# fims9000/SYNT_ISIC

Hardware: AMD Instinct MI355X
Metric: images/sec at 3x64x64 T=1000 (DDPM reverse-diffusion sampling) (higher is better)
Workload: dtype f32

## Files before the change

### synt_isic_amd/csrc/common.h

```cpp
#pragma once

#include <hip/hip_runtime.h>

#include <atomic>
#include <cstdarg>
#include <cstdint>
#include <cstdio>
#include <string>
#include <map>
#include <mutex>
#include <vector>

#include "../../include/sisic.h"

namespace sisic {

void set_error(const char* fmt, ...);

#define SISIC_HIP(call)                                                                   \
    do {                                                                                  \
        hipError_t _e = (call);                                                           \
        if (_e != hipSuccess) {                                                           \
            ::sisic::set_error("%s failed: %s (%s:%d)", #call, hipGetErrorString(_e),     \
                               __FILE__, __LINE__);                                       \
// ... 41 lines not shown
    std::map<hipStream_t, SplitK> splitk;
    std::mutex splitk_mutex;
    struct Bf3Items { int key[9]; unsigned* tab = nullptr; hipStream_t fill_stream = nullptr; hipEvent_t fill_done = nullptr; };
    std::vector<Bf3Items> bf3_items;
    std::mutex bf3_items_mutex;
    std::atomic<uint64_t> scratch_generation{0};
};

namespace sisic {

struct ProfileScope {
    sisic_ctx* ctx;
    hipStream_t stream;
    PendingEvent ev{};
    bool active = false;
    ProfileScope(sisic_ctx* c, hipStream_t s, int kind, double bytes, double flops, double flops_exec = -1.0, int kind2 = -1);
    ~ProfileScope();
};

int profile_collect(sisic_ctx* ctx);

inline int ensure_dynamic_lds(sisic_ctx* ctx, const void* kern, int bytes, std::atomic<uint64_t>& done) {
    const uint64_t bit = uint64_t(1) << (ctx->device & 63);
    if (done.load(std::memory_order_acquire) & bit) return SISIC_OK;
    SISIC_HIP(hipFuncSetAttribute(kern, hipFuncAttributeMaxDynamicSharedMemorySize, bytes));
    done.fetch_or(bit, std::memory_order_release);
    return SISIC_OK;
}

inline int cdiv(int a, int b) { return (a + b - 1) / b; }
inline int wino_latency_ksplit(int Cout, int Cin, int Hout, int Wout) {
    const int co_t = Cout > 64 ? 128 : 64;
    const int per_image = cdiv(Hout, 8) * cdiv(Wout, 16) * cdiv(Cout, co_t);
    const int nchunks = cdiv(Cin, 8);
    int k = 1;
    while (per_image * k < 256 && k < 8 && nchunks % (2 * k) == 0) k *= 2;
    return k;
}
inline int wino_latency_segments(int Hout, int Wout) { return cdiv(Hout * Wout, 1024); }
inline int64_t cdiv64(int64_t a, int64_t b) { return (a + b - 1) / b; }
inline int round_up(int a, int b) { return cdiv(a, b) * b; }

constexpr int CONV_CO_TILE = 64;
inline int conv_ci_chunk(int ksize) { return ksize == 1 ? 32 : (ksize == 3 ? 16 : 4); }
inline int conv_cin_pad(int cin, int ksize) { return round_up(cin, conv_ci_chunk(ksize)); }
inline int conv_cout_pad(int cout) { return round_up(cout, CONV_CO_TILE); }
inline int64_t conv_packed_floats(int cout, int cin, int ksize) {
    const int64_t first = (int64_t)conv_cin_pad(cin, ksize) * ksize * ksize * conv_cout_pad(cout);
    return ksize == 1 ? 3 * first + first / 2 : first;
}

int launch_conv2d(sisic_ctx*, const sisic_conv_args& a, hipStream_t s);
int launch_conv_smallcout(sisic_ctx*, const sisic_conv_args& a, hipStream_t s);
int launch_score_head_bwd(sisic_ctx*, const float* logits, const float* fc_w, const float* act, float* g, int B, int C,
                          int HW, int n_classes, int target, hipStream_t s);
int launch_relu_bwd(sisic_ctx*, const float* dy, const float* y, float* out, int64_t n, hipStream_t s);
int launch_scatter_add_even(sisic_ctx*, float* dst, const float* src, int planes, int H, int W, hipStream_t s);
int launch_maxpool_bwd(sisic_ctx*, const float* dm, const float* xin, float* dx, int planes, int H, int W, hipStream_t s);
int launch_stem_bwd(sisic_ctx*, const float* g, const float* w_oihw, float* dp, int B, int CO, int OH, int OW, int H, int W,
                    hipStream_t s);
int launch_preprocess_bwd(sisic_ctx*, const float* dp, const float* x, float* dx, int B, int H, int W, int OH, int OW,
                          hipStream_t s);
int launch_add_relu(sisic_ctx*, const float* y, const float* identity, float* out, int64_t n, hipStream_t s);
int launch_gradcam(sisic_ctx*, const float* y, const float* outp, const float* fc_w, const float* bias, float* cam, int B, int C,
                   int h, int w, int S, int target, hipStream_t s);
int conv_stats_slots(const sisic_conv_args& a);
bool conv_finalizes(const sisic_conv_args& a);
bool conv_pointwise_applicable(const sisic_conv_args& a);
int conv_pointwise_stats_slots(const sisic_conv_args& a);
int launch_conv_pointwise(sisic_ctx*, const sisic_conv_args& a, hipStream_t s);
bool conv_pointwise_bf3_applicable(const sisic_conv_args& a);
int launch_conv_pointwise_bf3(sisic_ctx*, const sisic_conv_args& a, hipStream_t s);
bool conv_s2_bf3_applicable(const sisic_conv_args& a);
int conv_s2_bf3_stats_slots(const sisic_conv_args& a);
int launch_conv_s2_bf3(sisic_ctx*, const sisic_conv_args& a, hipStream_t s);
int64_t conv_s2_packed_floats(int Cout, int Cin);
int launch_conv_s2_pack(sisic_ctx*, const float* w, int Cout, int Cin, float* out, hipStream_t s);
int launch_gn_finalize(sisic_ctx*, const float* st0, int c0, int slots0, const float* st1, int c1, int slots1, int B,
                       int HW, int groups, float eps, const float* gamma, const float* beta, float* scale, float* shift,
                       hipStream_t s, float* mean_rstd = nullptr);
int launch_conv_winograd(sisic_ctx*, const sisic_conv_args& a, const float* u_packed, int cfg, hipStream_t s);
int launch_winograd_pack(sisic_ctx*, const float* w, int Cout, int Cin, float* packed, hipStream_t s);
int64_t winograd_packed_numel(int Cout, int Cin);
inline int64_t winograd_first_floats(int Cout, int Cin) { return (int64_t)round_up(Cin, 16) * 16 * conv_cout_pad(Cout); }
int launch_conv_pack(sisic_ctx*, const float* w, int Cout, int Cin, int k, float* packed, hipStream_t s);
int launch_gn_stats(sisic_ctx*, const float* in0, int c0, const float* in1, int c1, int B, int HW, int groups,
                    float eps, const float* gamma, const float* beta, float* scale, float* shift, hipStream_t s,
                    float* mean_rstd = nullptr);
int launch_attention(sisic_ctx*, const float* qkv, float* out, int B, int C, int N, int head_dim, hipStream_t s);
int launch_ddpm_step(sisic_ctx*, const float* eps, const float* x, const float* z, float* out, int64_t n,
                     float sb, float sa, float c0, float c1, float sigma, float clip, hipStream_t s);
size_t loop_state_bytes();
int launch_loop_select_row(sisic_ctx*, const float* table, int R, const void* state, float* out, hipStream_t s);
int launch_loop_advance(sisic_ctx*, void* state, hipStream_t s);
int launch_ddpm_step_indexed(sisic_ctx*, const float* eps, float* x, int64_t n, const void* state, const float* coef,
                             const int* zrow, float clip, hipStream_t s);
int launch_ddpm_step_rng(sisic_ctx*, const float* eps, const float* x, float* out, int64_t n, int64_t n_per_image,
                         const uint64_t* seeds_dev, uint32_t step, float sb, float sa, float c0, float c1, float sigma,
                         float clip, hipStream_t s);
int launch_ddpm_step_indexed_rng(sisic_ctx*, const float* eps, float* x, int64_t n, int64_t n_per_image, const void* state,
                                 const float* coef, const uint64_t* seeds_dev, float clip, hipStream_t s);
int launch_noise_fill(sisic_ctx*, void* out, int B, int64_t n_per_image, const uint64_t* seeds_host, uint32_t step,
                      uint32_t tag, bool bits, hipStream_t s);
int launch_denorm_u8(sisic_ctx*, const float* x, uint8_t* out, int B, int C, int H, int W, hipStream_t s, int form = 0);
int launch_temb_mlp(sisic_ctx*, const float* t_vals, int B, const float* freqs, int n_freqs, const float* w1t,
                    const float* b1, const float* w2t, const float* b2, int hidden, float* temb_act, hipStream_t s,
// ... 29 lines not shown
```

### synt_isic_amd/csrc/conv_mfma.hip

```cpp
#include <cstdlib>
#include <type_traits>

#include "common.h"
#include "pack_device.h"

namespace sisic {

typedef float f32x16 __attribute__((ext_vector_type(16)));

struct ConvParams {
    const float* in0;
    const float* in1;
    int c0, c1;
    int B, Hin, Win;
    int Hc, Wc;
    int Hout, Wout;
    int ups;
    int zero_insert;
    const float* w;
    int cout_pad;
    const float* bias;
    int Cout;
    const float* gn_scale;
    const float* gn_shift;
// ... 354 lines not shown
                                 float* __restrict__ out) {
    const size_t first = (size_t)cin_pad * KK * cout_pad;
    const size_t total = KK == 1 ? 3 * first + first / 2 : first;
    for (size_t i = (size_t)blockIdx.x * blockDim.x + threadIdx.x; i < total; i += (size_t)gridDim.x * blockDim.x) {
        conv_pack_elem(i, w, Cout, Cin, KK, cin_pad, cout_pad, out);
    }
}

template <int KS, int STRIDE, int MT, int NT, int WM, int WN, int TW, int CIC, int OCC = 2, int KSP = 1>
static int launch_cfg(sisic_ctx* ctx, ConvParams& p, hipStream_t s) {
    using G = ConvGeom<KS, STRIDE, MT, NT, WM, WN, TW, CIC, KSP>;
    p.tiles_x = cdiv(p.Wout, TW);
    p.tiles_y = cdiv(p.Hout, G::TH);
    p.n_co_tiles = p.cout_pad / G::CO_TILE;
    p.nchunks = cdiv(p.c0 + p.c1, CIC);
    const int64_t nwg = (int64_t)p.B * p.tiles_x * p.tiles_y * p.n_co_tiles;
    SISIC_REQUIRE(nwg > 0 && nwg < (int64_t(1) << 31), "conv2d: grid of %lld workgroups unsupported", (long long)nwg);
    p.nwg = (int)nwg;
    if (p.slots_query) {
        *p.slots_query = p.tiles_x * p.tiles_y * WN;
        return SISIC_OK;
    }
    if constexpr (KS == 1 && STRIDE == 1 && TW == G::PIX && G::EPT % 4 == 0) {
        const bool aligned = ((reinterpret_cast<uintptr_t>(p.in0) | reinterpret_cast<uintptr_t>(p.in1)) & 15) == 0;
        if (p.Wc % 4 == 0 && aligned) {
            auto kern4 = conv_mfma_kernel<KS, STRIDE, MT, NT, WM, WN, TW, CIC, OCC, KSP, true>;
            static std::atomic<uint64_t> lds_opt_in4{0};
            SISIC_TRY(ensure_dynamic_lds(ctx, reinterpret_cast<const void*>(kern4), (int)G::LDS_BYTES, lds_opt_in4));
            hipLaunchKernelGGL(kern4, dim3(p.nwg), dim3(G::NTHR), G::LDS_BYTES, s, p);
            SISIC_HIP(hipGetLastError());
            return SISIC_OK;
        }
    }
    auto kern = conv_mfma_kernel<KS, STRIDE, MT, NT, WM, WN, TW, CIC, OCC, KSP>;
    static std::atomic<uint64_t> lds_opt_in{0};
    SISIC_TRY(ensure_dynamic_lds(ctx, reinterpret_cast<const void*>(kern), (int)G::LDS_BYTES, lds_opt_in));
    hipLaunchKernelGGL(kern, dim3(p.nwg), dim3(G::NTHR), G::LDS_BYTES, s, p);
    SISIC_HIP(hipGetLastError());
    return SISIC_OK;
}

int launch_conv_pack(sisic_ctx*, const float* w, int Cout, int Cin, int k, float* packed, hipStream_t s) {
    SISIC_REQUIRE(k == 1 || k == 3 || k == 7, "conv_pack: ksize %d unsupported", k);
    const int cin_pad = conv_cin_pad(Cin, k), cout_pad = conv_cout_pad(Cout);
    const size_t total = (size_t)cin_pad * k * k * cout_pad;
    const int blocks = (int)std::min<size_t>((total * (k == 1 ? 4 : 1) + 255) / 256, 4096);
    hipLaunchKernelGGL(conv_pack_kernel, dim3(blocks), dim3(256), 0, s, w, Cout, Cin, k * k, cin_pad, cout_pad, packed);
    SISIC_HIP(hipGetLastError());
    return SISIC_OK;
}

static int dispatch_conv2d(sisic_ctx* ctx, const sisic_conv_args& a, hipStream_t s, int* slots_query);

static int winograd_cfg(const sisic_conv_args& a) {
    if (!(a.ksize == 3 && a.stride == 1 && a.w_winograd != nullptr && a.Cout > 4) || a.upsample == 2) return 0;
    if ((a.tile_cfg >= 60 && a.tile_cfg <= 74) || a.tile_cfg == 78 || a.tile_cfg == 79 || (a.tile_cfg >= 90 && a.tile_cfg <= 92)) return a.tile_cfg;
    if (a.tile_cfg != 0) return 0;
    const int Hout = a.Hin << (a.upsample ? 1 : 0), Wout = a.Win << (a.upsample ? 1 : 0);
    const bool fits32 = 16.0 * std::max(a.c0, a.c1) * a.Hin * a.Win < 4294967296.0;
    if (!fits32) return 0;
    if (Hout >= 12 && Wout >= 12) {
        static const bool wide_on = [] { const char* e = std::getenv("SISIC_WINO_WIDE"); return !e || std::atoi(e) != 0; }();
        static const bool bf3_on = [] { const char* e = std::getenv("SISIC_WINO_BF16X3"); return !e || std::atoi(e) != 0; }();
        const int th = (Hout + 15) / 16 * 16, tw = (Wout + 15) / 16 * 16;
        if (bf3_on && a.Cout % 64 == 0 && 4 * Hout * Wout >= 3 * th * tw && a.c0 + a.c1 >= 16 &&
            a.c0 + a.c1 <= 2048 &&
            4.0 * a.Cout * Hout * Wout < 2147483648.0)
            return 74;
        if (wide_on && !a.upsample) return a.Cout > 64 ? 68 : 69;
        return 66;
    }
    const int Cin = a.c0 + a.c1;
    static const bool ksplit_on = [] { const char* e = std::getenv("SISIC_KSPLIT"); return !e || std::atoi(e) != 0; }();
    if (ksplit_on && Hout <= 8 && Wout <= 8 && Hout >= 5 && Wout >= 5 && Cin >= 128 && Cin % 32 == 0 && a.Cout >= 128) {
        static const bool wide_on = [] { const char* e = std::getenv("SISIC_WINO_WIDE"); return !e || std::atoi(e) != 0; }();
        static const bool bf3_on = [] { const char* e = std::getenv("SISIC_WINO_BF16X3"); return !e || std::atoi(e) != 0; }();
        if (bf3_on && !a.upsample && a.Cout % 64 == 0 && Cin <= 512) return 92;
        return (wide_on && !a.upsample) ? 91 : 90;
    }
    return 0;
}
static bool winograd_selected(const sisic_conv_args& a) { return winograd_cfg(a) != 0; }

int conv_stats_slots(const sisic_conv_args& a) {
    if (const int cfg = winograd_cfg(a)) {
        if (cfg >= 90 && cfg <= 92) return 1;
        const int Hout = a.Hin << (a.upsample ? 1 : 0), Wout = a.Win << (a.upsample ? 1 : 0);
        if ((cfg == 78 || cfg == 79) && wino_latency_ksplit(a.Cout, a.c0 + a.c1, Hout, Wout) > 1) return wino_latency_segments(Hout, Wout);
        if ((cfg >= 68 && cfg <= 73) || cfg == 78 || cfg == 79) return ((Hout + 7) / 8) * ((Wout + 15) / 16);
        const int edge = (cfg == 61 || cfg == 63 || cfg == 65 || cfg == 67) ? 8 : 16;
        return ((Hout + edge - 1) / edge) * ((Wout + edge - 1) / edge);
    }
    int slots = 0;
    sisic_conv_args q = a;
    q.stats_out = nullptr;
    if (dispatch_conv2d(nullptr, q, nullptr, &slots) != SISIC_OK) return 0;
    return slots;
}

bool conv_finalizes(const sisic_conv_args& a) {
    if (!a.fin_gamma || a.fin_groups <= 0) return false;
    const int cfg = winograd_cfg(a);
    const int Hout = a.Hin << (a.upsample ? 1 : 0), Wout = a.Win << (a.upsample ? 1 : 0);
    if (a.Cout % a.fin_groups != 0 || a.Cout / a.fin_groups != 8) return false;
    if (cfg == 74) return !a.upsample && Hout <= 16 && Wout <= 16 && a.Cout % 64 == 0;
    if (cfg < 90 || cfg > 92) return false;
    if (Hout * Wout != 64 || a.Cout % 16 != 0) return false;
    return ((reinterpret_cast<uintptr_t>(a.residual) | reinterpret_cast<uintptr_t>(a.out) | reinterpret_cast<uintptr_t>(a.stats_out)) & 15) == 0;
}

int launch_conv2d(sisic_ctx* ctx, const sisic_conv_args& a, hipStream_t s) { return dispatch_conv2d(ctx, a, s, nullptr); }

static int dispatch_conv2d(sisic_ctx* ctx, const sisic_conv_args& a, hipStream_t s, int* slots_query) {
    SISIC_REQUIRE(a.in0 && a.w_packed && a.out, "conv2d: null tensor");
    SISIC_REQUIRE(a.B > 0 && a.Hin > 0 && a.Win > 0 && a.c0 > 0 && a.c1 >= 0 && a.Cout > 0, "conv2d: bad shape");
    SISIC_REQUIRE((a.c1 == 0) == (a.in1 == nullptr), "conv2d: in1/c1 mismatch");
    SISIC_REQUIRE(a.ksize == 1 || a.ksize == 3 || a.ksize == 7, "conv2d: ksize %d unsupported", a.ksize);
    SISIC_REQUIRE(a.stride == 1 || a.stride == 2, "conv2d: stride %d unsupported", a.stride);
    SISIC_REQUIRE(a.ksize != 7 || a.stride == 2, "conv2d: 7x7 is built for stride 2 only (the ResNet stem)");
    SISIC_REQUIRE(!(a.upsample && a.stride != 1), "conv2d: upsample with stride");
    SISIC_REQUIRE((a.gn_scale == nullptr) == (a.gn_shift == nullptr), "conv2d: gn_scale/gn_shift mismatch");

    ConvParams p{};
    p.in0 = a.in0; p.in1 = a.in1; p.c0 = a.c0; p.c1 = a.c1;
    p.B = a.B; p.Hin = a.Hin; p.Win = a.Win;
    p.ups = a.upsample ? 1 : 0;
    p.zero_insert = a.upsample == 2 ? 1 : 0;
    p.Hc = a.Hin << p.ups; p.Wc = a.Win << p.ups;
    const int pad = a.ksize / 2;
    p.Hout = (p.Hc + 2 * pad - a.ksize) / a.stride + 1;
    p.Wout = (p.Wc + 2 * pad - a.ksize) / a.stride + 1;
    p.w = a.w_packed; p.cout_pad = conv_cout_pad(a.Cout);
    p.bias = a.bias; p.Cout = a.Cout;
    p.gn_scale = a.gn_scale; p.gn_shift = a.gn_shift; p.gn_silu = a.gn_silu;
    p.chan_bias = a.chan_bias; p.chan_bias_stride = a.chan_bias_stride; p.residual = a.residual; p.relu = a.relu; p.out = a.out;
    p.stats = a.stats_out; p.slots_query = slots_query;

    const int Cin = a.c0 + a.c1;
    const double kk = double(a.ksize) * a.ksize;
    const double out_elems = double(a.B) * a.Cout * p.Hout * p.Wout;
    const double bytes = 4.0 * (double(a.B) * Cin * a.Hin * a.Win + out_elems) + 4.0 * (Cin * a.Cout * kk + a.Cout) +
                         (a.residual ? 4.0 * out_elems : 0.0);
    const double flops = 2.0 * out_elems * Cin * kk;
    int cfg = a.tile_cfg;
    const bool use_wino = winograd_selected(a);
    SISIC_REQUIRE(a.stats_out == nullptr || conv_stats_slots(a) > 0,
                  "conv2d: stats_out given but sisic_conv_stats_slots() is 0 for these arguments");
    const bool wino_ups9 = use_wino && a.upsample && !a.gn_scale && winograd_cfg(a) == 66;
    ProfileScope prof(slots_query ? nullptr : ctx, s, a.ksize == 1 ? PK_CONV1 : PK_CONV3, bytes, flops,
                      use_wino ? flops * (wino_ups9 ? 9.0 : 16.0) / 36.0 : flops,
                      (use_wino && winograd_cfg(a) == 74) ? PK_WINO_BF3 :
                      (use_wino && !wino_ups9 && (winograd_cfg(a) == 66 || (winograd_cfg(a) >= 68 && winograd_cfg(a) <= 73) || winograd_cfg(a) == 78 || winograd_cfg(a) == 79)) ? PK_WINO_MAIN : -1);

    if (a.ksize == 3 && a.stride == 1 && !a.upsample && a.Cout <= 4 && (cfg == 0 || (cfg >= 50 && cfg <= 52))) {
        if (slots_query) return SISIC_OK;
        return launch_conv_smallcout(ctx, a, s);
    }
    if (use_wino) {
        SISIC_REQUIRE(!slots_query, "conv2d: internal: slot query on the Winograd path");
        return launch_conv_winograd(ctx, a, a.w_winograd, winograd_cfg(a), s);
    }
    SISIC_REQUIRE((cfg < 60 || cfg > 74) && cfg != 78 && cfg != 79 && (cfg < 90 || cfg > 92), "conv2d: tile_cfg %d needs w_winograd, ksize 3 and stride 1", cfg);
    if (a.ksize == 7) {
        if (cfg == 0) cfg = 41;
        if (cfg == 41) return launch_cfg<7, 2, 2, 1, 1, 4, 32, 2>(ctx, p, s);
        if (cfg == 42) return launch_cfg<7, 2, 2, 1, 1, 4, 32, 4>(ctx, p, s);
    } else if (a.ksize == 1 && a.stride == 2) {
        if (cfg == 0) cfg = p.Wout >= 24 ? 31 : (p.Wout >= 12 ? 32 : 33);
        switch (cfg) {
            case 31: return launch_cfg<1, 2, 2, 1, 1, 4, 32, 16>(ctx, p, s);
            case 32: return launch_cfg<1, 2, 2, 1, 1, 4, 16, 16>(ctx, p, s);
            case 33: return launch_cfg<1, 2, 1, 1, 2, 2, 8, 16>(ctx, p, s);
        }
    } else if (a.ksize == 1) {
        p.Hin = 1; p.Win = a.Hin * a.Win; p.Hc = 1; p.Wc = p.Win; p.Hout = 1; p.Wout = p.Win; p.ups = 0;
        SISIC_REQUIRE(!a.upsample, "conv2d: 1x1 with upsample");
        static const bool pw_on = [] { const char* e = std::getenv("SISIC_POINTWISE"); return !e || std::atoi(e) != 0; }();
        static const bool pwb_on = [] { const char* e = std::getenv("SISIC_POINTWISE_BF16X3"); return !e || std::atoi(e) != 0; }();
        if ((cfg == 0 && pwb_on && conv_pointwise_bf3_applicable(a)) || (cfg >= 28 && cfg <= 30) || cfg == 34 || cfg == 35) {
            if (slots_query) { *slots_query = conv_pointwise_stats_slots(a); return SISIC_OK; }
            return launch_conv_pointwise_bf3(ctx, a, s);
        }
        if ((cfg == 0 && pw_on && conv_pointwise_applicable(a)) || cfg == 20) {
            if (slots_query) { *slots_query = conv_pointwise_stats_slots(a); return SISIC_OK; }
            return launch_conv_pointwise(ctx, a, s);
        }
        if (cfg == 0) cfg = (p.Wout <= 64) ? 22 : (p.Wout <= 256 ? 25 : 24);
        switch (cfg) {
            case 21: return launch_cfg<1, 1, 2, 2, 1, 4, 256, 16>(ctx, p, s);
            case 22: return launch_cfg<1, 1, 1, 1, 2, 2, 64, 16>(ctx, p, s);
            case 23: return launch_cfg<1, 1, 2, 1, 1, 4, 128, 16>(ctx, p, s);
            case 24: return launch_cfg<1, 1, 1, 2, 2, 4, 256, 32, 4>(ctx, p, s);
            case 25: return launch_cfg<1, 1, 1, 1, 2, 4, 128, 32, 4>(ctx, p, s);
            case 26: return launch_cfg<1, 1, 1, 2, 2, 4, 256, 16, 4>(ctx, p, s);
            case 27: return launch_cfg<1, 1, 1, 1, 2, 4, 128, 16, 4>(ctx, p, s);
        }
    } else if (a.stride == 1) {
        if (cfg == 0) cfg = p.Wout >= 24 ? 8 : (p.Wout >= 12 ? 9 : 16);
        switch (cfg) {
            case 1: return launch_cfg<3, 1, 2, 2, 1, 4, 64, 8>(ctx, p, s);
            case 2: return launch_cfg<3, 1, 2, 2, 1, 4, 32, 8>(ctx, p, s);
            case 3: return launch_cfg<3, 1, 2, 2, 1, 4, 16, 8>(ctx, p, s);
            case 4: return launch_cfg<3, 1, 1, 1, 2, 2, 8, 8>(ctx, p, s);
            case 16: return launch_cfg<3, 1, 1, 1, 2, 2, 8, 16, 2, 2>(ctx, p, s);
            case 17: return launch_cfg<3, 1, 1, 1, 2, 2, 8, 8, 2, 2>(ctx, p, s);
            case 5: return launch_cfg<3, 1, 2, 1, 1, 4, 16, 8>(ctx, p, s);
            case 6: return launch_cfg<3, 1, 2, 1, 1, 4, 64, 8>(ctx, p, s);
// ... 28 lines not shown
```

### synt_isic_amd/csrc/conv_small.hip

```cpp
#include <atomic>
#include <type_traits>

#include "common.h"

namespace sisic {

constexpr int CS_TW = 32, CS_PX = 4, CS_CIC = 2;
constexpr int CS_IW = CS_TW + 2;
constexpr int CS_IWP = 36;
template <int CS_TH>
struct CSGeom;
template <int CS_TH, int KS>
constexpr size_t cs_lds_bytes();
template <int CS_TH>
struct CSGeom {
    static constexpr int THR = (CS_TW / CS_PX) * CS_TH;
    static constexpr int IH = CS_TH + 2;
    static constexpr int TPC = THR / CS_CIC;
    static constexpr int EPT = (IH * CS_IWP + TPC - 1) / TPC;
    static constexpr int CHS = EPT * TPC;
    static_assert(CS_IWP >= CS_IW + 2 && CS_IWP % 4 == 0 && CHS % 4 == 0, "aligned rows");
    static_assert(CS_CIC * 9 <= THR, "one thread per filter row");
};

template <int CS_TH, int KS>
constexpr size_t cs_lds_bytes() {
    constexpr size_t in = (size_t)KS * 2 * CS_CIC * CSGeom<CS_TH>::CHS, red = (size_t)(KS - 1) * CS_PX * 4 * CSGeom<CS_TH>::THR;
    return sizeof(float) * (in > red ? in : red);
}

struct ConvSmallParams {
    const float* in0;
    const float* in1;
    int c0, c1, B, H, W;
    const float* w;
    int cout_pad;
    const float* bias;
    int Cout;
    const float* gn_scale;
    const float* gn_shift;
    int gn_silu;
    const float* chan_bias;
    int chan_bias_stride;
    const float* residual;
    int relu;
    float* out;
    int tiles_x, tiles_y, nchunks;
};

template <int CS_TH, int KS>
__global__ void __launch_bounds__(CSGeom<CS_TH>::THR * KS, KS == 1 ? 3 : 4) conv3x3_smallcout_kernel(const ConvSmallParams p) {
    constexpr int CS_THR = CSGeom<CS_TH>::THR, CS_IH = CSGeom<CS_TH>::IH, CS_TPC = CSGeom<CS_TH>::TPC, CS_EPT = CSGeom<CS_TH>::EPT,
                  CS_CHS = CSGeom<CS_TH>::CHS;
    constexpr int IN_FLOATS = 2 * CS_CIC * CS_CHS, RED_FLOATS = (KS - 1) * CS_PX * 4 * CS_THR;
    extern __shared__ __attribute__((aligned(16))) float lds_all[];
    __shared__ __attribute__((aligned(16))) float w_all[KS][2][CS_CIC * 9 * 4];
    const int grp = KS == 1 ? 0 : __builtin_amdgcn_readfirstlane((int)threadIdx.x / CS_THR);
    float (*in_lds)[CS_CIC * CS_CHS] = reinterpret_cast<float (*)[CS_CIC * CS_CHS]>(lds_all + grp * IN_FLOATS);
    float (*w_lds)[CS_CIC * 9 * 4] = w_all[grp];

    int tile = blockIdx.x;
    const int tx = tile % p.tiles_x;
    tile /= p.tiles_x;
    const int ty = tile % p.tiles_y;
    const int b = tile / p.tiles_y;
    const int oy0 = ty * CS_TH, ox0 = tx * CS_TW;
    const int tid = threadIdx.x - grp * CS_THR;
    const int sci = tid / CS_TPC, sl = tid % CS_TPC;
    const int HW = p.H * p.W, Cin = p.c0 + p.c1;
    const int prologue = (p.gn_scale == nullptr) ? 0 : (p.gn_silu ? 2 : 1);
    const int n_mine = p.nchunks / KS, c_first = grp * n_mine;

    int goff[CS_EPT];
    unsigned vmask = 0;
#pragma unroll
    for (int i = 0; i < CS_EPT; ++i) {
        const int e = sl + i * CS_TPC;
        const int yy = e / CS_IWP, xx = e % CS_IWP;
        const int gy = oy0 - 1 + yy, gx = ox0 - 1 + xx;
        const bool v = yy < CS_IH && xx < CS_IW && gy >= 0 && gy < p.H && gx >= 0 && gx < p.W;
        goff[i] = v ? gy * p.W + gx : 0;
        vmask |= (v ? 1u : 0u) << i;
    }

    float rin[CS_EPT];
    float rw[4];
    float gsc = 1.0f, gsh = 0.0f;
    bool cval = false;

    auto load_chunk = [&](int chunk) {
        const int c = chunk * CS_CIC + sci;
        cval = c < Cin;
        const int cc = min(c, Cin - 1);
        const float* src = (cc < p.c0) ? p.in0 + ((size_t)b * p.c0 + cc) * HW : p.in1 + ((size_t)b * p.c1 + (cc - p.c0)) * HW;
#pragma unroll
        for (int i = 0; i < CS_EPT; ++i) rin[i] = src[goff[i]];
        if (prologue) {
            gsc = p.gn_scale[(size_t)b * Cin + cc];
            gsh = p.gn_shift[(size_t)b * Cin + cc];
        }
        const int row = min(tid, CS_CIC * 9 - 1);
        const float4 t = *reinterpret_cast<const float4*>(p.w + ((size_t)chunk * CS_CIC * 9 + row) * p.cout_pad);
        rw[0] = t.x; rw[1] = t.y; rw[2] = t.z; rw[3] = t.w;
    };
    auto store_chunk = [&](int buf) {
        float* dst = &in_lds[buf][sci * CS_CHS + sl];
        const unsigned m = cval ? vmask : 0u;
#pragma unroll
        for (int i = 0; i < CS_EPT; ++i) {
            float v = rin[i];
            if (prologue) v = v * gsc + gsh;
            if (prologue == 2) v = v * __builtin_amdgcn_rcpf(1.0f + __expf(-v));
            dst[i * CS_TPC] = ((m >> i) & 1u) ? v : 0.0f;
        }
        if (tid < CS_CIC * 9) *reinterpret_cast<float4*>(&w_lds[buf][tid * 4]) = make_float4(rw[0], rw[1], rw[2], rw[3]);
    };

    const int py = tid / (CS_TW / CS_PX), px0 = (tid % (CS_TW / CS_PX)) * CS_PX;
    float acc[CS_PX][4];
#pragma unroll
    for (int q = 0; q < CS_PX; ++q)
#pragma unroll
        for (int co = 0; co < 4; ++co) acc[q][co] = 0.0f;
    load_chunk(c_first);
    store_chunk(0);
    __syncthreads();
    for (int k = 0; k < n_mine; ++k) {
        const int chunk = c_first + k;
        const int buf = k & 1;
        const bool more = k + 1 < n_mine;
        if (more) load_chunk(chunk + 1);
        const float* I = &in_lds[buf][py * CS_IWP + px0];
        const float* Wt = &w_lds[buf][0];
#pragma unroll 1
        for (int ci = 0; ci < CS_CIC; ++ci) {
#pragma unroll
            for (int ky = 0; ky < 3; ++ky) {
                const float* row = I + ci * CS_CHS + ky * CS_IWP;
                const float4 r4 = *reinterpret_cast<const float4*>(row);
                const float2 r2 = *reinterpret_cast<const float2*>(row + 4);
                const float in[6] = {r4.x, r4.y, r4.z, r4.w, r2.x, r2.y};
#pragma unroll
                for (int kx = 0; kx < 3; ++kx) {
                    const float4 w4 = *reinterpret_cast<const float4*>(&Wt[(ci * 9 + ky * 3 + kx) * 4]);
#pragma unroll
                    for (int q = 0; q < CS_PX; ++q) {
                        const float a = in[q + kx];
                        acc[q][0] += a * w4.x; acc[q][1] += a * w4.y; acc[q][2] += a * w4.z; acc[q][3] += a * w4.w;
                    }
                }
            }
        }
        if (more) store_chunk(buf ^ 1);
        __syncthreads();
    }
    if constexpr (KS > 1) {
        if (grp > 0) {
#pragma unroll
            for (int q = 0; q < CS_PX; ++q)
#pragma unroll
                for (int co = 0; co < 4; ++co) lds_all[((grp - 1) * CS_PX * 4 + q * 4 + co) * CS_THR + tid] = acc[q][co];
        }
        __syncthreads();
        if (grp > 0) return;
#pragma unroll
        for (int g = 1; g < KS; ++g)
#pragma unroll
            for (int q = 0; q < CS_PX; ++q)
#pragma unroll
                for (int co = 0; co < 4; ++co) acc[q][co] += lds_all[((g - 1) * CS_PX * 4 + q * 4 + co) * CS_THR + tid];
    }

    const int oy = oy0 + py, ox = ox0 + px0;
    if (oy < p.H) {
        const bool vec = (p.W & 3) == 0;
#pragma unroll
        for (int co = 0; co < 4; ++co) {
            if (co < p.Cout) {
                const size_t base = ((size_t)b * p.Cout + co) * HW + (size_t)oy * p.W;
                float add = 0.0f;
                if (p.bias) add += p.bias[co];
                if (p.chan_bias) add += p.chan_bias[(size_t)b * p.chan_bias_stride + co];
                float v[CS_PX];
#pragma unroll
                for (int q = 0; q < CS_PX; ++q) {
                    v[q] = acc[q][co] + add;
                    if (p.residual && ox + q < p.W) v[q] += p.residual[base + ox + q];
                    if (p.relu) v[q] = fmaxf(v[q], 0.0f);
                }
                if (vec) {
                    if (ox < p.W) *reinterpret_cast<float4*>(p.out + base + ox) = make_float4(v[0], v[1], v[2], v[3]);
                } else {
#pragma unroll
                    for (int q = 0; q < CS_PX; ++q)
                        if (ox + q < p.W) p.out[base + ox + q] = v[q];
                }
            }
        }
    }
}

int launch_conv_smallcout(sisic_ctx* ctx, const sisic_conv_args& a, hipStream_t s) {
    ConvSmallParams p{};
    p.in0 = a.in0; p.in1 = a.in1; p.c0 = a.c0; p.c1 = a.c1; p.B = a.B; p.H = a.Hin; p.W = a.Win;
    p.w = a.w_packed; p.cout_pad = conv_cout_pad(a.Cout); p.bias = a.bias; p.Cout = a.Cout;
    p.gn_scale = a.gn_scale; p.gn_shift = a.gn_shift; p.gn_silu = a.gn_silu;
    p.chan_bias = a.chan_bias; p.chan_bias_stride = a.chan_bias_stride; p.residual = a.residual; p.relu = a.relu;
    p.out = a.out;
    p.tiles_x = cdiv(a.Win, CS_TW);
    p.nchunks = cdiv(a.c0 + a.c1, CS_CIC);
    const bool spare = a.tile_cfg == 50 || (a.tile_cfg != 51 && (int64_t)a.B * p.tiles_x * cdiv(a.Hin, 32) >= 256);
    p.tiles_y = cdiv(a.Hin, spare ? 32 : 8);
    const int64_t nwg = (int64_t)a.B * p.tiles_x * p.tiles_y;
    SISIC_REQUIRE(nwg > 0 && nwg < (int64_t(1) << 31), "conv2d(small): grid too large");
    const bool ksplit = a.tile_cfg != 52 && p.nchunks % 4 == 0 && p.nchunks >= 16;
    auto go = [&](auto th_tag, auto ks_tag) -> int {
        constexpr int TH = decltype(th_tag)::value, KSV = decltype(ks_tag)::value;
        auto kern = conv3x3_smallcout_kernel<TH, KSV>;
        static std::atomic<uint64_t> opt{0};
        SISIC_TRY(ensure_dynamic_lds(ctx, reinterpret_cast<const void*>(kern), (int)(cs_lds_bytes<TH, KSV>()), opt));
        constexpr size_t lds = cs_lds_bytes<TH, KSV>();
        constexpr unsigned thr = (unsigned)(CSGeom<TH>::THR * KSV);
        hipLaunchKernelGGL(kern, dim3((unsigned)nwg), dim3(thr), lds, s, p);
        return SISIC_OK;
    };
    using I = std::integral_constant<int, 1>;
    if (ksplit) {
        if (spare) SISIC_TRY(go(std::integral_constant<int, 32>{}, std::integral_constant<int, 4>{}));
        else SISIC_TRY(go(std::integral_constant<int, 8>{}, std::integral_constant<int, 4>{}));
    } else {
        if (spare) SISIC_TRY(go(std::integral_constant<int, 32>{}, I{}));
        else SISIC_TRY(go(std::integral_constant<int, 8>{}, I{}));
    }
    SISIC_HIP(hipGetLastError());
    return SISIC_OK;
}

}
```

Before: 11.68.

## Add direct small-Cin input conv kernel and packed-FMA small-Cout output conv

Adds a dedicated direct 3x3 convolution kernel for layers with at most four input channels and Cout divisible by 64, such as the UNet input conv. It holds the input window in registers and uses packed two-wide FMAs over output channels, and it can emit fused GroupNorm statistics. Before, this layer went through the Winograd/MFMA path. The small-Cout output-conv kernel also gains a channel-interleaved LDS layout, so two input channels are computed with packed FMAs per output channel, plus a 16-row tile option. Both paths are on by default with environment switches to disable them, and they add template instantiations and new edge-case handling.

```diff
diff --git a/synt_isic_amd/csrc/common.h b/synt_isic_amd/csrc/common.h
--- a/synt_isic_amd/csrc/common.h
+++ b/synt_isic_amd/csrc/common.h
@@ -117,6 +117,9 @@
 
 int launch_conv2d(sisic_ctx*, const sisic_conv_args& a, hipStream_t s);
 int launch_conv_smallcout(sisic_ctx*, const sisic_conv_args& a, hipStream_t s);
+bool conv_smallcin_applicable(const sisic_conv_args& a);
+int conv_smallcin_stats_slots(const sisic_conv_args& a);
+int launch_conv_smallcin(sisic_ctx*, const sisic_conv_args& a, hipStream_t s);
 int launch_score_head_bwd(sisic_ctx*, const float* logits, const float* fc_w, const float* act, float* g, int B, int C,
                           int HW, int n_classes, int target, hipStream_t s);
 int launch_relu_bwd(sisic_ctx*, const float* dy, const float* y, float* out, int64_t n, hipStream_t s);
diff --git a/synt_isic_amd/csrc/conv_mfma.hip b/synt_isic_amd/csrc/conv_mfma.hip
--- a/synt_isic_amd/csrc/conv_mfma.hip
+++ b/synt_isic_amd/csrc/conv_mfma.hip
@@ -430,7 +430,13 @@
 
 static int dispatch_conv2d(sisic_ctx* ctx, const sisic_conv_args& a, hipStream_t s, int* slots_query);
 
+static bool smallcin_selected(const sisic_conv_args& a) {
+    static const bool direct_on = [] { const char* e = std::getenv("SISIC_CONV_IN_DIRECT"); return !e || std::atoi(e) != 0; }();
+    return (a.tile_cfg == 53 || (a.tile_cfg == 0 && direct_on)) && conv_smallcin_applicable(a);
+}
+
 static int winograd_cfg(const sisic_conv_args& a) {
+    if (smallcin_selected(a)) return 0;
     if (!(a.ksize == 3 && a.stride == 1 && a.w_winograd != nullptr && a.Cout > 4) || a.upsample == 2) return 0;
     if ((a.tile_cfg >= 60 && a.tile_cfg <= 74) || a.tile_cfg == 78 || a.tile_cfg == 79 || (a.tile_cfg >= 90 && a.tile_cfg <= 92)) return a.tile_cfg;
     if (a.tile_cfg != 0) return 0;
@@ -530,7 +536,12 @@
                       (use_wino && winograd_cfg(a) == 74) ? PK_WINO_BF3 :
                       (use_wino && !wino_ups9 && (winograd_cfg(a) == 66 || (winograd_cfg(a) >= 68 && winograd_cfg(a) <= 73) || winograd_cfg(a) == 78 || winograd_cfg(a) == 79)) ? PK_WINO_MAIN : -1);
 
-    if (a.ksize == 3 && a.stride == 1 && !a.upsample && a.Cout <= 4 && (cfg == 0 || (cfg >= 50 && cfg <= 52))) {
+    if (smallcin_selected(a)) {
+        if (slots_query) { *slots_query = conv_smallcin_stats_slots(a); return SISIC_OK; }
+        return launch_conv_smallcin(ctx, a, s);
+    }
+    SISIC_REQUIRE(cfg != 53, "conv2d: tile_cfg 53 needs ksize 3, stride 1, one source of <= 4 channels, no prologue, Cout %% 64 == 0");
+    if (a.ksize == 3 && a.stride == 1 && !a.upsample && a.Cout <= 4 && (cfg == 0 || (cfg >= 50 && cfg <= 52) || cfg == 54 || cfg == 55)) {
         if (slots_query) return SISIC_OK;
         return launch_conv_smallcout(ctx, a, s);
     }
diff --git a/synt_isic_amd/csrc/conv_small.hip b/synt_isic_amd/csrc/conv_small.hip
--- a/synt_isic_amd/csrc/conv_small.hip
+++ b/synt_isic_amd/csrc/conv_small.hip
@@ -1,10 +1,13 @@
 #include <atomic>
+#include <cstdlib>
 #include <type_traits>
 
 #include "common.h"
 
 namespace sisic {
 
+typedef float cs_v2f __attribute__((ext_vector_type(2)));
+typedef float cs_v4f __attribute__((ext_vector_type(4)));
 constexpr int CS_TW = 32, CS_PX = 4, CS_CIC = 2;
 constexpr int CS_IW = CS_TW + 2;
 constexpr int CS_IWP = 36;
@@ -48,8 +51,8 @@
     int tiles_x, tiles_y, nchunks;
 };
 
-template <int CS_TH, int KS>
-__global__ void __launch_bounds__(CSGeom<CS_TH>::THR * KS, KS == 1 ? 3 : 4) conv3x3_smallcout_kernel(const ConvSmallParams p) {
+template <int CS_TH, int KS, int CO>
+__global__ void __launch_bounds__(CSGeom<CS_TH>::THR * KS, (KS == 1 || (CO == 0 && CS_TH == 8)) ? 3 : 4) conv3x3_smallcout_kernel(const ConvSmallParams p) {
     constexpr int CS_THR = CSGeom<CS_TH>::THR, CS_IH = CSGeom<CS_TH>::IH, CS_TPC = CSGeom<CS_TH>::TPC, CS_EPT = CSGeom<CS_TH>::EPT,
                   CS_CHS = CSGeom<CS_TH>::CHS;
     constexpr int IN_FLOATS = 2 * CS_CIC * CS_CHS, RED_FLOATS = (KS - 1) * CS_PX * 4 * CS_THR;
@@ -66,21 +69,20 @@
     const int b = tile / p.tiles_y;
     const int oy0 = ty * CS_TH, ox0 = tx * CS_TW;
     const int tid = threadIdx.x - grp * CS_THR;
-    const int sci = tid / CS_TPC, sl = tid % CS_TPC;
+    const int sci = (CS_TPC % 64 == 0) ? __builtin_amdgcn_readfirstlane(tid / CS_TPC) : tid / CS_TPC, sl = tid % CS_TPC;
     const int HW = p.H * p.W, Cin = p.c0 + p.c1;
     const int prologue = (p.gn_scale == nullptr) ? 0 : (p.gn_silu ? 2 : 1);
     const int n_mine = p.nchunks / KS, c_first = grp * n_mine;
 
     int goff[CS_EPT];
-    unsigned vmask = 0;
+    bool inside[CS_EPT];
 #pragma unroll
     for (int i = 0; i < CS_EPT; ++i) {
         const int e = sl + i * CS_TPC;
         const int yy = e / CS_IWP, xx = e % CS_IWP;
         const int gy = oy0 - 1 + yy, gx = ox0 - 1 + xx;
-        const bool v = yy < CS_IH && xx < CS_IW && gy >= 0 && gy < p.H && gx >= 0 && gx < p.W;
-        goff[i] = v ? gy * p.W + gx : 0;
-        vmask |= (v ? 1u : 0u) << i;
+        inside[i] = yy < CS_IH && xx < CS_IW && gy >= 0 && gy < p.H && gx >= 0 && gx < p.W;
+        goff[i] = inside[i] ? (gy * p.W + gx) * (int)sizeof(float) : 0;
     }
 
     float rin[CS_EPT];
@@ -92,36 +94,55 @@
         const int c = chunk * CS_CIC + sci;
         cval = c < Cin;
         const int cc = min(c, Cin - 1);
-        const float* src = (cc < p.c0) ? p.in0 + ((size_t)b * p.c0 + cc) * HW : p.in1 + ((size_t)b * p.c1 + (cc - p.c0)) * HW;
-#pragma unroll
-        for (int i = 0; i < CS_EPT; ++i) rin[i] = src[goff[i]];
+        const bool first = cc < p.c0;
+        const size_t plane = first ? (size_t)b * p.c0 + cc : (size_t)b * p.c1 + (cc - p.c0);
+        const float* src = (first ? p.in0 : p.in1) + plane * HW;
+        if (cval) {
+#pragma unroll
+            for (int i = 0; i < CS_EPT; ++i) rin[i] = *reinterpret_cast<const float*>(reinterpret_cast<const char*>(src) + goff[i]);
+        } else {
+#pragma unroll
+            for (int i = 0; i < CS_EPT; ++i) rin[i] = 0.0f;
+        }
         if (prologue) {
-            gsc = p.gn_scale[(size_t)b * Cin + cc];
-            gsh = p.gn_shift[(size_t)b * Cin + cc];
+            gsc = cval ? p.gn_scale[(size_t)b * Cin + cc] : 0.0f;
+            gsh = cval ? p.gn_shift[(size_t)b * Cin + cc] : 0.0f;
         }
         const int row = min(tid, CS_CIC * 9 - 1);
         const float4 t = *reinterpret_cast<const float4*>(p.w + ((size_t)chunk * CS_CIC * 9 + row) * p.cout_pad);
         rw[0] = t.x; rw[1] = t.y; rw[2] = t.z; rw[3] = t.w;
     };
     auto store_chunk = [&](int buf) {
-        float* dst = &in_lds[buf][sci * CS_CHS + sl];
-        const unsigned m = cval ? vmask : 0u;
+        float* dst = CO > 0 ? &in_lds[buf][sl * CS_CIC + sci] : &in_lds[buf][sci * CS_CHS + sl];
+        constexpr int DS = CO > 0 ? CS_TPC * CS_CIC : CS_TPC;
 #pragma unroll
         for (int i = 0; i < CS_EPT; ++i) {
             float v = rin[i];
             if (prologue) v = v * gsc + gsh;
             if (prologue == 2) v = v * __builtin_amdgcn_rcpf(1.0f + __expf(-v));
-            dst[i * CS_TPC] = ((m >> i) & 1u) ? v : 0.0f;
-        }
-        if (tid < CS_CIC * 9) *reinterpret_cast<float4*>(&w_lds[buf][tid * 4]) = make_float4(rw[0], rw[1], rw[2], rw[3]);
+            dst[i * DS] = inside[i] ? v : 0.0f;
+        }
+        if (tid < CS_CIC * 9) {
+            if constexpr (CO > 0) {
+#pragma unroll
+                for (int co = 0; co < 4; ++co) w_lds[buf][((tid % 9) * 4 + co) * CS_CIC + tid / 9] = rw[co];
+            } else {
+                *reinterpret_cast<float4*>(&w_lds[buf][tid * 4]) = make_float4(rw[0], rw[1], rw[2], rw[3]);
+            }
+        }
     };
 
     const int py = tid / (CS_TW / CS_PX), px0 = (tid % (CS_TW / CS_PX)) * CS_PX;
     float acc[CS_PX][4];
+    cs_v2f acc2[CO > 0 ? CO : 1][CS_PX];
 #pragma unroll
     for (int q = 0; q < CS_PX; ++q)
 #pragma unroll
         for (int co = 0; co < 4; ++co) acc[q][co] = 0.0f;
+#pragma unroll
+    for (int co = 0; co < (CO > 0 ? CO : 1); ++co)
+#pragma unroll
+        for (int q = 0; q < CS_PX; ++q) acc2[co][q] = cs_v2f{0.0f, 0.0f};
     load_chunk(c_first);
     store_chunk(0);
     __syncthreads();
@@ -130,8 +151,36 @@
         const int buf = k & 1;
         const bool more = k + 1 < n_mine;
         if (more) load_chunk(chunk + 1);
+        const float* Wt = &w_lds[buf][0];
+        if constexpr (CO > 0) {
+            static_assert(CS_CIC == 2, "a packed FMA takes the chunk's two channels");
+            const float* I = &in_lds[buf][(py * CS_IWP + px0) * CS_CIC];
+#pragma unroll 1
+            for (int ky = 0; ky < 3; ++ky) {
+                const float* row = I + ky * CS_IWP * CS_CIC;
+                const cs_v4f ra = *reinterpret_cast<const cs_v4f*>(row);
+                const cs_v4f rb = *reinterpret_cast<const cs_v4f*>(row + 4);
+                const cs_v4f rc = *reinterpret_cast<const cs_v4f*>(row + 8);
+                const cs_v2f in[6] = {ra.xy, ra.zw, rb.xy, rb.zw, rc.xy, rc.zw};
+#pragma unroll
+                for (int kx = 0; kx < 3; ++kx) {
+                    const float* wt = &Wt[(ky * 3 + kx) * 4 * CS_CIC];
+                    cs_v2f wp[4];
+                    const cs_v4f wa = *reinterpret_cast<const cs_v4f*>(wt);
+                    wp[0] = wa.xy; wp[1] = wa.zw;
+                    if constexpr (CO == 3) wp[2] = *reinterpret_cast<const cs_v2f*>(wt + 4);
+                    if constexpr (CO == 4) {
+                        const cs_v4f wb = *reinterpret_cast<const cs_v4f*>(wt + 4);
+                        wp[2] = wb.xy; wp[3] = wb.zw;
+                    }
+#pragma unroll
+                    for (int co = 0; co < CO; ++co)
+#pragma unroll
+                        for (int q = 0; q < CS_PX; ++q) acc2[co][q] = __builtin_elementwise_fma(in[q + kx], wp[co], acc2[co][q]);
+                }
+            }
+        } else {
         const float* I = &in_lds[buf][py * CS_IWP + px0];
-        const float* Wt = &w_lds[buf][0];
 #pragma unroll 1
         for (int ci = 0; ci < CS_CIC; ++ci) {
 #pragma unroll
@@ -151,8 +200,15 @@
                 }
             }
         }
+        }
         if (more) store_chunk(buf ^ 1);
         __syncthreads();
+    }
+    if constexpr (CO > 0) {
+#pragma unroll
+        for (int q = 0; q < CS_PX; ++q)
+#pragma unroll
+            for (int co = 0; co < CO; ++co) acc[q][co] = acc2[co][q].x + acc2[co][q].y;
     }
     if constexpr (KS > 1) {
         if (grp > 0) {
@@ -209,14 +265,17 @@
     p.out = a.out;
     p.tiles_x = cdiv(a.Win, CS_TW);
     p.nchunks = cdiv(a.c0 + a.c1, CS_CIC);
-    const bool spare = a.tile_cfg == 50 || (a.tile_cfg != 51 && (int64_t)a.B * p.tiles_x * cdiv(a.Hin, 32) >= 256);
-    p.tiles_y = cdiv(a.Hin, spare ? 32 : 8);
+    const bool spare = a.tile_cfg == 50 || (a.tile_cfg != 51 && a.tile_cfg != 55 && (int64_t)a.B * p.tiles_x * cdiv(a.Hin, 32) >= 256);
+    const int th = a.tile_cfg == 55 ? 16 : (spare ? 32 : 8);
+    p.tiles_y = cdiv(a.Hin, th);
     const int64_t nwg = (int64_t)a.B * p.tiles_x * p.tiles_y;
     SISIC_REQUIRE(nwg > 0 && nwg < (int64_t(1) << 31), "conv2d(small): grid too large");
     const bool ksplit = a.tile_cfg != 52 && p.nchunks % 4 == 0 && p.nchunks >= 16;
-    auto go = [&](auto th_tag, auto ks_tag) -> int {
-        constexpr int TH = decltype(th_tag)::value, KSV = decltype(ks_tag)::value;
-        auto kern = conv3x3_smallcout_kernel<TH, KSV>;
+    static const bool packed_on = [] { const char* e = std::getenv("SISIC_CONV_OUT_STREAM"); return !e || std::atoi(e) != 0; }();
+    const int co_form = (a.tile_cfg == 54 || !packed_on) ? 0 : a.Cout;
+    auto go = [&](auto th_tag, auto ks_tag, auto co_tag) -> int {
+        constexpr int TH = decltype(th_tag)::value, KSV = decltype(ks_tag)::value, COV = decltype(co_tag)::value;
+        auto kern = conv3x3_smallcout_kernel<TH, KSV, COV>;
         static std::atomic<uint64_t> opt{0};
         SISIC_TRY(ensure_dynamic_lds(ctx, reinterpret_cast<const void*>(kern), (int)(cs_lds_bytes<TH, KSV>()), opt));
         constexpr size_t lds = cs_lds_bytes<TH, KSV>();
@@ -224,13 +283,23 @@
         hipLaunchKernelGGL(kern, dim3((unsigned)nwg), dim3(thr), lds, s, p);
         return SISIC_OK;
     };
-    using I = std::integral_constant<int, 1>;
-    if (ksplit) {
-        if (spare) SISIC_TRY(go(std::integral_constant<int, 32>{}, std::integral_constant<int, 4>{}));
-        else SISIC_TRY(go(std::integral_constant<int, 8>{}, std::integral_constant<int, 4>{}));
-    } else {
-        if (spare) SISIC_TRY(go(std::integral_constant<int, 32>{}, I{}));
-        else SISIC_TRY(go(std::integral_constant<int, 8>{}, I{}));
+    auto tiling = [&](auto co_tag) -> int {
+        using I = std::integral_constant<int, 1>;
+        if (ksplit) {
+            if (th == 32) return go(std::integral_constant<int, 32>{}, std::integral_constant<int, 4>{}, co_tag);
+            if (th == 16) return go(std::integral_constant<int, 16>{}, std::integral_constant<int, 4>{}, co_tag);
+            return go(std::integral_constant<int, 8>{}, std::integral_constant<int, 4>{}, co_tag);
+        }
+        if (th == 32) return go(std::integral_constant<int, 32>{}, I{}, co_tag);
+        if (th == 16) return go(std::integral_constant<int, 16>{}, I{}, co_tag);
+        return go(std::integral_constant<int, 8>{}, I{}, co_tag);
+    };
+    switch (co_form) {
+        case 1: SISIC_TRY(tiling(std::integral_constant<int, 1>{})); break;
+        case 2: SISIC_TRY(tiling(std::integral_constant<int, 2>{})); break;
+        case 3: SISIC_TRY(tiling(std::integral_constant<int, 3>{})); break;
+        case 4: SISIC_TRY(tiling(std::integral_constant<int, 4>{})); break;
+        default: SISIC_TRY(tiling(std::integral_constant<int, 0>{})); break;
     }
     SISIC_HIP(hipGetLastError());
     return SISIC_OK;
diff --git a/synt_isic_amd/csrc/conv_smallcin.hip b/synt_isic_amd/csrc/conv_smallcin.hip
--- /dev/null
+++ b/synt_isic_amd/csrc/conv_smallcin.hip
@@ -0,0 +1,220 @@
+#include "common.h"
+
+namespace sisic {
+
+typedef float sc_v2f __attribute__((ext_vector_type(2)));
+typedef float sc_v4f __attribute__((ext_vector_type(4)));
+
+constexpr int SC_THR = 256, SC_PX = 4, SC_COG = 16, SC_COB = 8;
+
+struct ConvSmallCinParams {
+    int B, H, W, Cout, cout_pad;
+    const float* chan_bias;
+    int chan_bias_stride;
+    const float* residual;
+    int relu, vec;
+    float* out;
+    float* stats;
+    int tiles_x, tiles_y, cgroups;
+};
+
+__device__ __forceinline__ float sc_wave_sum(float v) {
+    v += __int_as_float(__builtin_amdgcn_update_dpp(0, __float_as_int(v), 0xB1, 0xf, 0xf, true));
+    v += __int_as_float(__builtin_amdgcn_update_dpp(0, __float_as_int(v), 0x4E, 0xf, 0xf, true));
+    v += __int_as_float(__builtin_amdgcn_update_dpp(0, __float_as_int(v), 0x141, 0xf, 0xf, true));
+    v += __int_as_float(__builtin_amdgcn_update_dpp(0, __float_as_int(v), 0x140, 0xf, 0xf, true));
+    const int r = __float_as_int(v);
+    return (__int_as_float(__builtin_amdgcn_readlane(r, 0)) + __int_as_float(__builtin_amdgcn_readlane(r, 16))) +
+           (__int_as_float(__builtin_amdgcn_readlane(r, 32)) + __int_as_float(__builtin_amdgcn_readlane(r, 48)));
+}
+
+template <int CIN, int TW>
+__global__ void __launch_bounds__(SC_THR, CIN == 4 ? 3 : 4) conv3x3_smallcin_kernel(const float* __restrict__ in, const float* __restrict__ w,
+                                                                     const float* __restrict__ bias, const ConvSmallCinParams p) {
+    constexpr int TPR = TW / SC_PX, TH = SC_THR / TPR, WROWS = 64 / TPR;
+    int t = blockIdx.x;
+    const int cg = t % p.cgroups;
+    t /= p.cgroups;
+    const int tx = t % p.tiles_x;
+    t /= p.tiles_x;
+    const int ty = t % p.tiles_y;
+    const int b = t / p.tiles_y;
+    const int tid = threadIdx.x, wave = __builtin_amdgcn_readfirstlane(tid >> 6);
+    const int oy = ty * TH + tid / TPR, ox = tx * TW + (tid % TPR) * SC_PX;
+    const int HW = p.H * p.W;
+
+    __shared__ __attribute__((aligned(16))) float wl[CIN * 9 * SC_COG];
+    for (int i = tid; i < CIN * 9 * SC_COG; i += SC_THR) wl[i] = w[(size_t)(i / SC_COG) * p.cout_pad + cg * SC_COG + i % SC_COG];
+
+    sc_v2f x[CIN][3][SC_PX / 2 + 1];
+#pragma unroll
+    for (int ci = 0; ci < CIN; ++ci)
+#pragma unroll
+        for (int ky = 0; ky < 3; ++ky) {
+            const int gy = oy - 1 + ky;
+            const bool rok = gy >= 0 && gy < p.H;
+            const float* row = in + ((size_t)b * CIN + ci) * HW + (size_t)(rok ? gy : 0) * p.W;
+            float r[SC_PX + 2];
+            if (p.vec) {
+                const float4 m = (rok && ox < p.W) ? *reinterpret_cast<const float4*>(row + ox) : make_float4(0.f, 0.f, 0.f, 0.f);
+                r[0] = (rok && ox > 0 && ox - 1 < p.W) ? row[ox - 1] : 0.0f;
+                r[1] = m.x; r[2] = m.y; r[3] = m.z; r[4] = m.w;
+                r[5] = (rok && ox + 4 < p.W) ? row[ox + 4] : 0.0f;
+            } else {
+#pragma unroll
+                for (int j = 0; j < SC_PX + 2; ++j) {
+                    const int gx = ox - 1 + j;
+                    r[j] = (rok && gx >= 0 && gx < p.W) ? row[gx] : 0.0f;
+                }
+            }
+#pragma unroll
+            for (int j = 0; j < SC_PX / 2 + 1; ++j) x[ci][ky][j] = sc_v2f{r[2 * j], r[2 * j + 1]};
+        }
+    __syncthreads();
+
+    const int wrows = min(max(p.H - (ty * TH + wave * WROWS), 0), WROWS), wcols = min(p.W - tx * TW, TW);
+    const float cnt = (float)(wrows * wcols);
+    const int slots = p.tiles_x * p.tiles_y * (SC_THR / 64), slot = (ty * p.tiles_x + tx) * (SC_THR / 64) + wave;
+    const float rcnt = cnt > 0.0f ? 1.0f / cnt : 0.0f;
+    const bool rowin = oy < p.H;
+    bool pin[SC_PX];
+#pragma unroll
+    for (int q = 0; q < SC_PX; ++q) pin[q] = rowin && ox + q < p.W;
+
+#pragma unroll 1
+    for (int cb = 0; cb < SC_COG / SC_COB; ++cb) {
+        const int co0 = cg * SC_COG + cb * SC_COB;
+#pragma unroll
+        for (int ci = 0; ci < CIN; ++ci)
+#pragma unroll
+            for (int ky = 0; ky < 3; ++ky)
+#pragma unroll
+                for (int j = 0; j < SC_PX / 2 + 1; ++j) asm volatile("" : "+v"(x[ci][ky][j]));
+        sc_v2f acc[SC_COB / 2][SC_PX];
+#pragma unroll
+        for (int cp = 0; cp < SC_COB / 2; ++cp)
+#pragma unroll
+            for (int q = 0; q < SC_PX; ++q) acc[cp][q] = sc_v2f{0.0f, 0.0f};
+#pragma unroll
+        for (int ci = 0; ci < CIN; ++ci)
+#pragma unroll
+            for (int ky = 0; ky < 3; ++ky) {
+#pragma unroll
+                for (int kx = 0; kx < 3; ++kx) {
+                    const int tap = ci * 9 + ky * 3 + kx;
+                    const sc_v4f wa = *reinterpret_cast<const sc_v4f*>(&wl[tap * SC_COG + cb * SC_COB]);
+                    const sc_v4f wb = *reinterpret_cast<const sc_v4f*>(&wl[tap * SC_COG + cb * SC_COB + 4]);
+                    const sc_v2f wv[SC_COB / 2] = {wa.xy, wa.zw, wb.xy, wb.zw};
+#pragma unroll
+                    for (int q = 0; q < SC_PX; ++q) {
+                        const int j = q + kx;
+                        const sc_v2f xj = x[ci][ky][j / 2];
+                        const sc_v2f a = (j & 1) ? __builtin_shufflevector(xj, xj, 1, 1) : __builtin_shufflevector(xj, xj, 0, 0);
+#pragma unroll
+                        for (int cp = 0; cp < SC_COB / 2; ++cp) acc[cp][q] = __builtin_elementwise_fma(a, wv[cp], acc[cp][q]);
+                    }
+                }
+            }
+#pragma unroll
+        for (int cp = 0; cp < SC_COB / 2; ++cp)
+#pragma unroll
+            for (int q = 0; q < SC_PX; ++q) asm volatile("" : "+v"(acc[cp][q]));
+#pragma unroll
+        for (int c = 0; c < SC_COB; ++c) {
+            const int co = co0 + c;
+            const size_t base = ((size_t)b * p.Cout + co) * HW + (size_t)(rowin ? oy : 0) * p.W + ox;
+            float add = 0.0f;
+            if (bias) add += bias[co];
+            if (p.chan_bias) add += p.chan_bias[(size_t)b * p.chan_bias_stride + co];
+            float v[SC_PX];
+#pragma unroll
+            for (int q = 0; q < SC_PX; ++q) v[q] = acc[c / 2][q][c % 2] + add;
+            if (p.residual) {
+                if (p.vec) {
+                    if (pin[0]) {
+                        const float4 r = *reinterpret_cast<const float4*>(p.residual + base);
+                        v[0] += r.x; v[1] += r.y; v[2] += r.z; v[3] += r.w;
+                    }
+                } else {
+#pragma unroll
+                    for (int q = 0; q < SC_PX; ++q)
+                        if (pin[q]) v[q] += p.residual[base + q];
+                }
+            }
+            if (p.relu) {
+#pragma unroll
+                for (int q = 0; q < SC_PX; ++q) v[q] = fmaxf(v[q], 0.0f);
+            }
+            if (p.vec) {
+                if (pin[0]) *reinterpret_cast<float4*>(p.out + base) = make_float4(v[0], v[1], v[2], v[3]);
+            } else {
+#pragma unroll
+                for (int q = 0; q < SC_PX; ++q)
+                    if (pin[q]) p.out[base + q] = v[q];
+            }
+            if (p.stats) {
+                const float K = __int_as_float(__builtin_amdgcn_readlane(__float_as_int(v[0]), 0));
+                float s1 = 0.0f, s2 = 0.0f;
+#pragma unroll
+                for (int q = 0; q < SC_PX; ++q) {
+                    const float d = pin[q] ? v[q] - K : 0.0f;
+                    s1 += d;
+                    s2 = fmaf(d, d, s2);
+                }
+                s1 = sc_wave_sum(s1);
+                s2 = sc_wave_sum(s2);
+                if ((tid & 63) == 0) {
+                    float4* dst = reinterpret_cast<float4*>(p.stats) + ((size_t)b * p.Cout + co) * slots + slot;
+                    *dst = cnt > 0.0f ? make_float4(cnt, fmaf(cnt, K, s1), fmaxf(s2 - s1 * s1 * rcnt, 0.0f), 0.0f)
+                                      : make_float4(0.f, 0.f, 0.f, 0.f);
+                }
+            }
+        }
+    }
+}
+
+bool conv_smallcin_applicable(const sisic_conv_args& a) {
+    return a.ksize == 3 && a.stride == 1 && !a.upsample && a.gn_scale == nullptr && a.c1 == 0 && a.in1 == nullptr && a.c0 >= 1 &&
+           a.c0 <= 4 && a.Cout % 64 == 0;
+}
+
+static int sc_tile_w(const sisic_conv_args& a) { return a.Win > 32 ? 64 : 32; }
+
+int conv_smallcin_stats_slots(const sisic_conv_args& a) {
+    const int tw = sc_tile_w(a);
+    return cdiv(a.Win, tw) * cdiv(a.Hin, SC_THR * SC_PX / tw) * (SC_THR / 64);
+}
+
+int launch_conv_smallcin(sisic_ctx* ctx, const sisic_conv_args& a, hipStream_t s) {
+    SISIC_REQUIRE(conv_smallcin_applicable(a), "conv2d(small-cin): needs ksize 3, stride 1, one source of <= 4 channels, no prologue, Cout %% 64 == 0");
+    ConvSmallCinParams p{};
+    p.B = a.B; p.H = a.Hin; p.W = a.Win; p.Cout = a.Cout; p.cout_pad = conv_cout_pad(a.Cout);
+    p.chan_bias = a.chan_bias; p.chan_bias_stride = a.chan_bias_stride; p.residual = a.residual; p.relu = a.relu;
+    p.out = a.out; p.stats = a.stats_out;
+    const uintptr_t ptrs = reinterpret_cast<uintptr_t>(a.in0) | reinterpret_cast<uintptr_t>(a.out) | reinterpret_cast<uintptr_t>(a.residual);
+    p.vec = ((a.Win & 3) == 0 && (ptrs & 15) == 0) ? 1 : 0;
+    const int tw = sc_tile_w(a);
+    p.tiles_x = cdiv(a.Win, tw); p.tiles_y = cdiv(a.Hin, SC_THR * SC_PX / tw); p.cgroups = a.Cout / SC_COG;
+    const int64_t nwg = (int64_t)a.B * p.tiles_x * p.tiles_y * p.cgroups;
+    SISIC_REQUIRE(nwg > 0 && nwg < (int64_t(1) << 31), "conv2d(small-cin): grid too large");
+    auto go = [&](auto kern) { hipLaunchKernelGGL(kern, dim3((unsigned)nwg), dim3(SC_THR), 0, s, a.in0, a.w_packed, a.bias, p); };
+    if (tw == 64) {
+        switch (a.c0) {
+            case 1: go(conv3x3_smallcin_kernel<1, 64>); break;
+            case 2: go(conv3x3_smallcin_kernel<2, 64>); break;
+            case 3: go(conv3x3_smallcin_kernel<3, 64>); break;
+            default: go(conv3x3_smallcin_kernel<4, 64>); break;
+        }
+    } else {
+        switch (a.c0) {
+            case 1: go(conv3x3_smallcin_kernel<1, 32>); break;
+            case 2: go(conv3x3_smallcin_kernel<2, 32>); break;
+            case 3: go(conv3x3_smallcin_kernel<3, 32>); break;
+            default: go(conv3x3_smallcin_kernel<4, 32>); break;
+        }
+    }
+    SISIC_HIP(hipGetLastError());
+    return SISIC_OK;
+}
+
+}
```

Result: no change. 11.70 (median of 6 runs) (+0.2%).
